# danielreardon/scintools

Hardware: NVIDIA B200
Metric: theta-theta eta-trials/sec on 4096x8192 dynspec (higher is better)
Workload: dtype f32

## Files before the change

### scintools_b200/csrc/api.cu

```cuda
#include <stdarg.h>
#include <string.h>

#include <vector>

#include "../../include/scint_b200.h"
#include "common.cuh"
#include "thth.cuh"

namespace sb {

static thread_local char g_err[512] = "";
static void* g_ws[8] = {nullptr};
static size_t g_ws_bytes[8] = {0};
static int g_sms = 148;

void set_error(const char* fmt, ...) {
    va_list ap;
    va_start(ap, fmt);
    vsnprintf(g_err, sizeof(g_err), fmt, ap);
    va_end(ap);
}
const char* last_error() { return g_err; }
int num_sms() { return g_sms; }

static long long g_launches = 0;
void count_launch() { ++g_launches; }

struct ProfPair { int id; cudaEvent_t a, b; };
static bool g_prof_on = false;
static std::vector<ProfPair> g_prof_pending;
static std::vector<cudaEvent_t> g_prof_pool;
static cudaEvent_t g_prof_open[PROF_COUNT];

static cudaEvent_t prof_event() {
    if (!g_prof_pool.empty()) {
        cudaEvent_t e = g_prof_pool.back();
        g_prof_pool.pop_back();
        return e;
    }
    cudaEvent_t e;
    cudaEventCreate(&e);
    return e;
}
void prof_begin(int id, cudaStream_t st) {
    if (!g_prof_on) return;
    g_prof_open[id] = prof_event();
    cudaEventRecord(g_prof_open[id], st);
}
void prof_end(int id, cudaStream_t st) {
    if (!g_prof_on) return;
    cudaEvent_t b = prof_event();
    cudaEventRecord(b, st);
    g_prof_pending.push_back({id, g_prof_open[id], b});
}

void* workspace(int slot, size_t bytes) {
    if (slot < 0 || slot >= 8) return nullptr;
    if (bytes <= g_ws_bytes[slot] && g_ws[slot]) return g_ws[slot];
    if (g_ws[slot]) {
        cudaDeviceSynchronize();
        cudaFree(g_ws[slot]);
        g_ws[slot] = nullptr;
        g_ws_bytes[slot] = 0;
    }
    size_t want = (bytes + (size_t(1) << 20) - 1) & ~((size_t(1) << 20) - 1);
    void* p = nullptr;
    cudaError_t e = cudaMalloc(&p, want);
    if (e != cudaSuccess) {
        set_error("workspace slot %d: cudaMalloc(%zu) -> %s", slot, want,
                  cudaGetErrorString(e));
        cudaGetLastError();
        return nullptr;
    }
    g_ws[slot] = p;
    g_ws_bytes[slot] = want;
    return p;
}

void workspace_release() {
    cudaDeviceSynchronize();
    for (int i = 0; i < 8; ++i) {
        if (g_ws[i]) cudaFree(g_ws[i]);
        g_ws[i] = nullptr;
        g_ws_bytes[i] = 0;
    }
}

int eta_sweep(const ThthGeom& g, const double* th_host, const double* d_etas,
              int neta, double tol, int max_iter, double* d_eigs,
              int* d_status, int* d_nred, int* d_iters, cudaStream_t st);
int thth_map(const ThthGeom& g, double eta, int hermitian, float2* d_out,
             int* d_tau_inv, int* d_fd_inv, unsigned char* d_pnts,
             unsigned char* d_th_pnts, int* d_err, cudaStream_t st);

int sspec(const float* dyn, int nf, int nt, const float* wt, const float* wf,
          double swt, double swf, int prewhite, int halve, int db,
          const float* pd1, const float* pd2, float* sec, cudaStream_t st,
          int noshift = 0);
int conj_spectrum(const float* dyn, int nf, int nt, int npad, float pad_value,
                  const unsigned char* rowmask, int half, long pitch, int ncols_keep,
                  float2* CS, cudaStream_t st);
int acf(const float* dyn, int nf, int nt, int subtract_mean, int normalise,
        float* out, cudaStream_t st);
int acf_sspec(const float* dyn, int nf, int nt, const float* wt, const float* wf,
              double swt, double swf, int normalise, float* out, cudaStream_t st);
void twiddle_release();
struct SimParams {
    int nx, ny;
    double dx, dy, alpha, ar, psi, inner, consp;
};
int sim_weights(const SimParams& p, double* w, cudaStream_t st);
int sim_screen(int nx, int ny, const double* w, const double* n1, const double* n2,
               unsigned long long seed, double* xyp, cudaStream_t st);
int sim_intensity(int nx, int ny, int nf, const double* xyp, const double* scales_host,
                  double ffconx, double ffcony, float2* spe_t, float* xyi,
                  cudaStream_t st);

template <typename A, typename B>
__global__ void convert_kernel(const A* __restrict__ a, B* __restrict__ b, long long n) {
    for (long long i = (long long)blockIdx.x * blockDim.x + threadIdx.x; i < n;
         i += (long long)gridDim.x * blockDim.x)
        b[i] = (B)a[i];
}

struct ThinGeom {
    ThthGeom g;
    const double* th2;
    int n2;
    double tau_max;
    double center_cut;
    int power;
};
int thin_sweep(const ThinGeom& t, const double* d_eta1, const double* d_eta2, int neta,
               double tol, int max_iter, double* d_sv, int* d_status, int* d_n1, int* d_n2,
               int* d_iters, cudaStream_t st);
int thin_map(const ThinGeom& t, double e1, double e2, float2* d_out, int* d_err,
             cudaStream_t st);

int rev_map(const float2* thth, int n, const double* th_dev, double eta, double tau0,
            double dtau, int ntau, double fd0, double dfd, int nfd, int hermitian,
            float2* recov, cudaStream_t st);
int herm_eigvec(const float2* A, int n, int ld, double tol, int max_iter, double* w_dev,
                float2* V_dev, int* info_dev, cudaStream_t st);
int ifft2_c2c(const float2* in, int n0, int n1, int centred, int crop0, int crop1,
              double scale, int real_only, void* out, cudaStream_t st);

int gerchberg_saxton(float2* W, const float* amp, const unsigned char* rowmask, int n0, int n1,
                     int niter, cudaStream_t st);

int conj_spectrum_bound(const float* dyn, int nf, int nt, int npad, float pad_value, float* out,
                        cudaStream_t st);
int norm_sspec_rows(const float* sspec, int nr, int nc, const double* fdop, const double* tdel,
                    double eta, double maxnormfac, const double* fdopnew, int nq, float* out,
                    double* power, cudaStream_t st);
int norm_sspec_avg(const float* norm, int nr, int nq, const double* weights, double* avg,
                   cudaStream_t st);
int scale_dyn_lambda(const float* dyn, int nf, int nt, int flip, const float* a,
                     const float* cp, const float* inv, const float* g, float p0, float pn,
                     const int* idx, const float4* W, int nlam, float* out, cudaStream_t st);

static int to_geom(const sb_thth_geom* in, ThthGeom* g) {
    SB_ARG(in != nullptr);
    SB_ARG(in->ntau > 0 && in->nfd > 0);
    SB_ARG(in->th_cents != nullptr && in->th_cents_host != nullptr);
    SB_ARG(in->n_th > 0);
    g->cs = (const float2*)in->cs;
    g->ntau = in->ntau;
    g->nfd = in->nfd;
    g->tau0 = in->tau0;
    g->dtau = in->dtau;
    g->half_dtau = in->dtau / 2;
    g->tau_absmax = in->tau_absmax;
    g->fd0 = in->fd0;
    g->dfd = in->dfd;
    g->half_dfd = in->dfd / 2;
    g->inv_dtau = 1.0 / in->dtau;
    g->inv_dfd = 1.0 / in->dfd;
    g->fd_half = in->fd_half;
    g->th = in->th_cents;
    g->n = in->n_th;
    g->coherent = in->coherent;
    g->cs_half = in->cs_half;
    g->cs_valid_cols = in->cs_half ? in->cs_valid_cols : 0;
    g->cs_bound = in->cs_bound;
    g->cs_pitch = in->cs_half ? in->cs_pitch : (in->cs_pitch > 0 ? in->cs_pitch : in->nfd);
    SB_ARG(!in->cs_half || (in->cs_pitch >= in->nfd / 2 + 1 && in->nfd % 2 == 0));
    return SB_OK;
}

}

extern "C" {

int sb_abi_version(void) { return 2; }
const char* sb_last_error(void) { return sb::last_error(); }

int sb_init(int device) {
    SB_CUDA(cudaSetDevice(device));
    SB_CUDA(cudaFree(0));
    cudaDeviceProp prop;
    SB_CUDA(cudaGetDeviceProperties(&prop, device));
    if (prop.major != 10) {
        sb::set_error("device %d is sm_%d%d; libscint_b200 is sm_100a only",
                      device, prop.major, prop.minor);
        return SB_ERR_UNSUPPORTED;
    }
    sb::g_sms = prop.multiProcessorCount;
    return SB_OK;
}

int64_t sb_launch_count(void) { return sb::g_launches; }

int sb_profile_enable(int32_t on) {
    sb::g_prof_on = on != 0;
    return SB_OK;
}

int sb_profile_collect(double* ms_host, int32_t* count_host, int32_t n) {
    SB_ARG(ms_host && count_host && n >= sb::PROF_COUNT);
    for (int i = 0; i < n; ++i) { ms_host[i] = 0.0; count_host[i] = 0; }
    SB_CUDA(cudaDeviceSynchronize());
    for (auto& p : sb::g_prof_pending) {
        float ms = 0.f;
        cudaEventElapsedTime(&ms, p.a, p.b);
        ms_host[p.id] += ms;
        count_host[p.id] += 1;
        sb::g_prof_pool.push_back(p.a);
        sb::g_prof_pool.push_back(p.b);
    }
    sb::g_prof_pending.clear();
    return SB_OK;
}

int sb_release(void) {
// ... 199 lines not shown
```

### scintools_b200/csrc/common.cuh

```cuda
#pragma once
#ifndef SB_HOST_EMU
#include <cuda_runtime.h>
#include <stdint.h>
#include <stdio.h>

#include "../../include/scint_b200.h"

namespace sb {

void set_error(const char* fmt, ...);
const char* last_error();

void* workspace(int slot, size_t bytes);
void workspace_release();
int num_sms();

enum ProfId { PROF_CS_ROWS = 0, PROF_CS_COLA, PROF_CS_COLB, PROF_THTH_PREP,
              PROF_THTH_BUILD, PROF_THTH_EIG, PROF_SSPEC, PROF_ACF, PROF_SIM_SCREEN,
              PROF_SIM_FREQ, PROF_COUNT };
void prof_begin(int id, cudaStream_t st);
void prof_end(int id, cudaStream_t st);
struct ProfScope {
    int id; cudaStream_t st;
    ProfScope(int i, cudaStream_t s) : id(i), st(s) { prof_begin(id, st); }
    ~ProfScope() { prof_end(id, st); }
};

#define SB_CUDA(call)                                                        \
    do {                                                                     \
        cudaError_t _e = (call);                                             \
        if (_e != cudaSuccess) {                                             \
            sb::set_error("%s:%d %s -> %s", __FILE__, __LINE__, #call,       \
                          cudaGetErrorString(_e));                           \
            return SB_ERR_CUDA;                                              \
        }                                                                    \
    } while (0)

void count_launch();

#define SB_LAUNCH_CHECK()                                                    \
    do {                                                                     \
        sb::count_launch();                                                  \
        cudaError_t _e = cudaGetLastError();                                 \
        if (_e != cudaSuccess) {                                             \
            sb::set_error("%s:%d launch -> %s", __FILE__, __LINE__,          \
                          cudaGetErrorString(_e));                           \
            return SB_ERR_CUDA;                                              \
        }                                                                    \
    } while (0)

#define SB_ARG(cond)                                                         \
    do {                                                                     \
        if (!(cond)) {                                                       \
            sb::set_error("%s:%d bad argument: %s", __FILE__, __LINE__,      \
                          #cond);                                            \
            return SB_ERR_ARG;                                               \
        }                                                                    \
    } while (0)

}
#endif

#ifdef SB_HOST_EMU
#define SB_SHARED static
#else
#define SB_SHARED __shared__
#endif

namespace sb {

__device__ __forceinline__ float warp_sum(float v) {
#pragma unroll
    for (int o = 16; o > 0; o >>= 1) v += __shfl_xor_sync(0xffffffffu, v, o);
    return v;
}
__device__ __forceinline__ double warp_sum(double v) {
#pragma unroll
    for (int o = 16; o > 0; o >>= 1) v += __shfl_xor_sync(0xffffffffu, v, o);
    return v;
}

__device__ __forceinline__ double floor_div_exact(double a, double b) {
    if (b > 0.0 && isfinite(a)) {
        double q = floor(__ddiv_rn(a, b));
        double r = __fma_rn(-q, b, a);
        if (r < 0.0) q -= 1.0;
        else if (r >= b) q += 1.0;
        return q;
    }
    if (b == 0.0) return __ddiv_rn(a, b);
    double mod = fmod(a, b);
    double div = __ddiv_rn(__dsub_rn(a, mod), b);
    if (mod != 0.0) {
        if ((b < 0.0) != (mod < 0.0)) div -= 1.0;
    }
    if (div != 0.0) {
        double fl = floor(div);
        if (div - fl > 0.5) fl += 1.0;
        return fl;
    }
    return copysign(0.0, __ddiv_rn(a, b));
}

__device__ __forceinline__ double floor_div_fast(double a, double b, double inv_b) {
    double q = floor(a * inv_b);
    if (b > 0.0 && fabs(q) < 1.0e15) {
        double r = __fma_rn(-q, b, a);
        if (r < 0.0) q -= 1.0;
        else if (r >= b) q += 1.0;
        return q;
    }
    return floor_div_exact(a, b);
}

}
```

### scintools_b200/csrc/thth.cu

```cuda
#include <float.h>
#include <limits.h>
#include <math.h>
#include <stdlib.h>

#include <type_traits>

#include "bf16_pack.cuh"
#include "lanczos.cuh"
#include "thth.cuh"
#include "tma.cuh"

namespace sb {

#ifndef SB_HOST_EMU
int eig_cluster_launch(const float2* d_M, int ld, int n_max, const int* d_nred, int e0,
                       int nb, double* d_eigs, int* d_status, int* d_iters, double tol,
                       double etol, int max_iter, cudaStream_t st);

int eig_half_launch(const float2* d_M, const unsigned* d_Mb, int ld, const int* d_nred, int e0,
                    int nb, double* d_eigs, int* d_status, int* d_iters, double tol, double etol,
                    int max_iter, bool tensor, cudaStream_t st);

#endif

enum { ST_OK = 0, ST_INDEX_ERROR = 1, ST_ZERO_START = 2, ST_TOO_SMALL = 4,
       ST_NOT_CONVERGED = 8 };

__global__ void thth_prep_kernel(ThthGeom g, const double* __restrict__ etas,
                                 int neta, int ld, int* __restrict__ idx,
                                 int* __restrict__ nred) {
    int e = blockIdx.x;
    if (e >= neta) return;
    double eta = etas[e];
    int lane = threadIdx.x;
    int base = 0;
    int* out = idx + (size_t)e * ld;
    for (int k0 = 0; k0 < g.n; k0 += 32) {
        int k = k0 + lane;
        bool keep = false;
        if (k < g.n) {
            double t = g.th[k];
            keep = (__dmul_rn(__dmul_rn(t, t), eta) < g.tau_absmax) &&
                   (fabs(t) < g.fd_half);
        }
        unsigned m = __ballot_sync(0xffffffffu, keep);
        if (keep) out[base + __popc(m & ((1u << lane) - 1u))] = k;
        base += __popc(m);
    }
    if (lane == 0) nred[e] = base;
}

__global__ void thth_indexerr_kernel(ThthGeom g, const double* __restrict__ etas,
                                     int* __restrict__ status) {
    int e = blockIdx.y;
    double eta = etas[e];
    long long total = (long long)g.n * g.n;
    bool bad = false;
    for (long long p = (long long)blockIdx.x * blockDim.x + threadIdx.x;
         p < total; p += (long long)gridDim.x * blockDim.x) {
        int i = (int)(p / g.n), j = (int)(p % g.n);
        ThthPoint pt = thth_point(g, eta, g.th[j], g.th[i]);
        bad |= pt.index_error;
    }
    if (__any_sync(0xffffffffu, bad) && (threadIdx.x & 31) == 0)
        atomicOr(status + e, ST_INDEX_ERROR);
}

#define SB_BUILD_EB 8

__device__ __forceinline__ unsigned pack_f16x2(float2 v) {
#ifdef SB_HOST_EMU
    const __half2 h = __floats2half2_rn(v.x, v.y);
    return (unsigned)h.x | ((unsigned)h.y << 16);
#else
    unsigned r;
    asm("cvt.rn.f16x2.f32 %0, %1, %2;" : "=r"(r) : "f"(v.y), "f"(v.x));
    return r;
#endif
}

__global__ void cs_absmax_kernel(const float2* __restrict__ cs, long long rows, long long ncols,
                                 long long pitch, unsigned* __restrict__ out) {
    float m = 0.f;
    const long long per_row4 = ncols >> 1;
    const long long total = rows * per_row4;
    for (long long i = (long long)blockIdx.x * blockDim.x + threadIdx.x; i < total;
         i += (long long)gridDim.x * blockDim.x) {
        const long long r = i / per_row4, c = i - r * per_row4;
        const float4 q = __ldg(reinterpret_cast<const float4*>(cs + r * pitch) + c);
        m = fmaxf(fmaxf(fmaxf(fabsf(q.x), fabsf(q.y)), fmaxf(fabsf(q.z), fabsf(q.w))), m);
    }
    if (ncols & 1) {
        for (long long r = (long long)blockIdx.x * blockDim.x + threadIdx.x; r < rows;
             r += (long long)gridDim.x * blockDim.x) {
            const float2 q = __ldg(cs + r * pitch + ncols - 1);
            m = fmaxf(fmaxf(fabsf(q.x), fabsf(q.y)), m);
        }
    }
    if (!(m == m)) m = 3.0e38f;
    m = fminf(m, 3.0e38f);
#pragma unroll
    for (int o = 16; o > 0; o >>= 1) m = fmaxf(m, __shfl_xor_sync(0xffffffffu, m, o));
    if ((threadIdx.x & 31) == 0) atomicMax(out, __float_as_uint(m));
}

template <int PACK, int ROWS, typename OFF>
__global__ void __launch_bounds__(32 * (32 / ROWS), ROWS == 8 ? 5 : 4)
thth_build_kernel(ThthGeom g, const double* __restrict__ etas, int eta0, int nbatch,
                  int ld, const int* __restrict__ idx,
                  const int* __restrict__ nred, float2* __restrict__ M,
                  unsigned* __restrict__ Mb, const unsigned* __restrict__ absmax, float span) {
    constexpr int TY = 32 / ROWS;
    int p = blockIdx.y, ta = 0;
    const int T = ld / 32;
    while (p >= T - ta) { p -= T - ta; ++ta; }
    const int tb = ta + p;
    const int tx = threadIdx.x, ty = threadIdx.y;
    const int b = tb * 32 + tx;
    const double ntau_d = (double)g.ntau;
    const long long hfd = g.nfd / 2;
    int cj = -2;
    double thj = 0.0;
    int ci[ROWS];
    double dk[ROWS];
    int col[ROWS];
    unsigned conj = 0u;
    float wk[ROWS];
#pragma unroll
    for (int k = 0; k < ROWS; ++k) { ci[k] = -2; dk[k] = 0.0; col[k] = -1; wk[k] = 0.f; }
    const int e_end = min(nbatch, (int)(blockIdx.x + 1) * SB_BUILD_EB);
    __shared__ float s_hscale[SB_BUILD_EB];
    if (PACK != 0) {
        const int lin = ty * 32 + tx;
        if (lin < SB_BUILD_EB) {
            const int e = blockIdx.x * SB_BUILD_EB + lin;
            float hs = 1.f;
            if (e < e_end) {
                const float seta = sqrtf((float)(2.0 * etas[eta0 + e]));
                const float bound = __uint_as_float(*absmax) * seta * sqrtf(span);
                if (bound > 0.f && bound < 3.0e38f) {
                    const float q = 32768.f / bound;
                    hs = q >= 1.1754944e-38f ? __uint_as_float(__float_as_uint(q) & 0x7f800000u) : 1.1754944e-38f;
                }
            }
            s_hscale[lin] = hs;
        }
        __syncthreads();
    }
    const unsigned foff0 = (unsigned)(ta * 32 + ty) * (unsigned)ld + (unsigned)b;
    const unsigned frow = (unsigned)TY * (unsigned)ld;
    const unsigned woff0 = ((unsigned)(2 * ta) * (unsigned)(ld >> 3) + (unsigned)(b >> 3)) * 128u +
                           (unsigned)ty * 8u;
    for (int e = blockIdx.x * SB_BUILD_EB; e < e_end; ++e) {
        const int n = nred[eta0 + e];
        if (tb * 32 >= n) continue;
        const double eta = etas[eta0 + e];
        const int* id = idx + (size_t)(eta0 + e) * ld;
        const int j = b < n ? id[b] : -1;
        if (j != cj) {
            cj = j;
            thj = j >= 0 ? g.th[j] : 0.0;
#pragma unroll
            for (int k = 0; k < ROWS; ++k) ci[k] = -2;
        }
        const float seta = sqrtf((float)(2.0 * eta));
        float2* Me = M + (size_t)e * ld * ld;
        const float hscale = PACK != 0 ? s_hscale[e - blockIdx.x * SB_BUILD_EB] : 1.f;
        OFF off[ROWS];
        unsigned hit = 0u;
#pragma unroll
        for (int k = 0; k < ROWS; ++k) {
            const int la = ty + TY * k;
            off[k] = 0;
            if (ta == tb && tx < la) continue;
            const int a = ta * 32 + la;
            const int i = a < n ? id[a] : -1;
            if (i != ci[k]) {
                ci[k] = i;
                col[k] = -1;
                conj &= ~(1u << k);
                wk[k] = 0.f;
                dk[k] = 0.0;
                if (i >= 0 && j > i && i + j != g.n - 1) {
                    const double th1 = thj, th2 = g.th[i];
                    dk[k] = __dsub_rn(__dmul_rn(th1, th1), __dmul_rn(th2, th2));
                    const double bb = __dadd_rn(__dsub_rn(__dsub_rn(th1, th2), g.fd0), g.half_dfd);
                    const double fqd = floor_div_fast(bb, g.dfd, g.inv_dfd);
                    const long long fq = (fqd == fqd && fabs(fqd) < 9.0e18) ? (long long)fqd : LLONG_MIN;
                    wk[k] = sqrtf((float)fabs(th2 - th1));
                    if (fq < g.nfd && !(fq < -g.nfd)) {
                        const long long fi = fq < 0 ? fq + g.nfd : fq;
                        if (!g.cs_half) col[k] = (int)fi;
                        else if (fi >= hfd) col[k] = (int)(fi - hfd);
                        else if (fi == 0) col[k] = (int)hfd;
                        else { col[k] = (int)(hfd - fi); conj |= 1u << k; }
                    }
                }
            }
            if (col[k] >= 0) {
                const double aa = __dadd_rn(__dsub_rn(__dmul_rn(eta, dk[k]), g.tau0), g.half_dtau);
                const double tqd = floor_div_fast(aa, g.dtau, g.inv_dtau);
                if (tqd > 0.0 && tqd < ntau_d) {
                    const int tq = (int)tqd;
                    const int r = (conj >> k) & 1u ? (int)g.ntau - tq : tq;
                    off[k] = (OFF)r * (OFF)g.cs_pitch + (OFF)col[k];
                    hit |= 1u << k;
                }
            }
        }
        float2 val[ROWS];
#pragma unroll
        for (int k = 0; k < ROWS; ++k) val[k] = __ldg(g.cs + off[k]);
#pragma unroll
        for (int k = 0; k < ROWS; ++k) {
            const int la = ty + TY * k;
            const bool low = ta == tb && tx < la;
            float2 v = make_float2(0.f, 0.f);
            if (!low) {
                if (col[k] >= 0) {
                    if ((hit >> k) & 1u) {
                        v = val[k];
                        if ((conj >> k) & 1u) v.y = -v.y;
                        if (!g.coherent) v = make_float2(hypotf(v.x, v.y), 0.f);
                    }
                    const float wf = seta * wk[k];
                    v.x *= wf;
                    v.y *= wf;
                    if (!(fabsf(v.x) <= 3.402823466e+38f) || !(fabsf(v.y) <= 3.402823466e+38f)) {
                        v.x = nan_to_num(v.x);
                        v.y = nan_to_num(v.y);
                    }
                }
                const unsigned o = foff0 + (unsigned)k * frow;
                Me[o] = v;
                if (PACK == 1) Mb[(size_t)e * ld * ld + o] = pack_f16x2(make_float2(v.x * hscale, v.y * hscale));
            }
            if (PACK == 2) {
                const unsigned h = low ? 0u : pack_f16x2(make_float2(v.x * hscale, v.y * hscale));
                const int i8 = tx & 7, s0 = (tx & ~7) + 2 * (i8 & 3);
                const unsigned ha = __shfl_sync(0xffffffffu, h, s0);
                const unsigned hb = __shfl_sync(0xffffffffu, h, s0 + 1);
                const unsigned word = i8 < 4 ? ((ha & 0xffffu) | (hb << 16)) : ((ha >> 16) | (hb & 0xffff0000u));
                if (!(ta == tb && (tx >> 4) < (la >> 4))) {
                    unsigned* Mw = Mb + (size_t)e * ld * ld;
                    const unsigned swz = (unsigned)(((la & 15) >> 2) & 1) << 2;
                    Mw[woff0 + (unsigned)(la >> 4) * (unsigned)(ld >> 3) * 128u + (unsigned)((la & 15) - ty) * 8u +
                       ((unsigned)i8 ^ swz)] = word;
                }
            }
        }
    }
}

template <int THREADS, bool TMA, int NST, bool FAST = false>
__global__ void __launch_bounds__(THREADS)
thth_eig_kernel(const float2* __restrict__ Mbase, int ld,
                const int* __restrict__ nred, int eta0,
                double* __restrict__ eigs, int* __restrict__ status,
                int* __restrict__ iters, double tol, double etol, int max_iter, int nb) {
    extern __shared__ __align__(128) unsigned char smem_raw[];
    constexpr int NW = THREADS / 32;
    LanczosShared& S = *reinterpret_cast<LanczosShared*>(smem_raw);
    float2* v = reinterpret_cast<float2*>(smem_raw + sizeof(LanczosShared));
    float2* vp = v + ld;
    float2* w = vp + ld;
    float2* u = w + ld;
    float4* stages = reinterpret_cast<float4*>(u + ld);
    float2* part = reinterpret_cast<float2*>(stages);
    unsigned long long* mbar = reinterpret_cast<unsigned long long*>(
        reinterpret_cast<unsigned char*>(stages) +
        (TMA ? (size_t)NW * NST * 4096 : (size_t)NW * 4096));
    const int tid = threadIdx.x, lane = tid & 31, warp = tid >> 5;
    if (TMA) {
        if (tid == 0) {
            for (int i = 0; i < NW * NST; ++i) mbar_init(mbar + i, 1);
            fence_mbarrier_init();
        }
    }
    unsigned gi = 0, gc = 0;
    for (int e = blockIdx.x; e < nb; e += gridDim.x) {
    __syncthreads();
    const int n = nred[eta0 + e];
    const float2* M = Mbase + (size_t)e * ld * ld;
    const double qnan = __longlong_as_double(0x7ff8000000000000LL);

    if (status[eta0 + e] & ST_INDEX_ERROR) {
        if (tid == 0) { eigs[eta0 + e] = qnan; iters[eta0 + e] = 0; }
        continue;
    }
    if (n < 3) {
        if (tid == 0) {
            eigs[eta0 + e] = qnan; iters[eta0 + e] = 0;
            status[eta0 + e] |= ST_TOO_SMALL;
        }
        continue;
    }
    const int h = n / 2;
    double part0 = 0.0;
    for (int c = tid; c < ld; c += THREADS) {
        float2 x = make_float2(0.f, 0.f);
        if (c < n && c > h) x = M[(size_t)h * ld + c];
        else if (c < h) { x = M[(size_t)c * ld + h]; x.y = -x.y; }
        v[c] = x;
        vp[c] = make_float2(0.f, 0.f);
        part0 += (double)x.x * x.x + (double)x.y * x.y;
    }
    part0 = warp_sum(part0);
    if (lane == 0) S.red[0][warp] = part0;
    if (tid == 0) {
        S.done = 0; S.lo = 0.0; S.theta = 0.0; S.res = 0.0; S.m_lo2 = 0; S.lo2 = 0.0;
        S.next_check = 1; S.m_last = 0; S.beta2[0] = 0.0;
    }
    __syncthreads();
    double nrm2 = 0.0;
    for (int k = 0; k < NW; ++k) nrm2 += S.red[0][k];
    if (!(nrm2 > 0.0) || !isfinite(nrm2)) {
        if (tid == 0) {
            eigs[eta0 + e] = qnan; iters[eta0 + e] = 0;
            status[eta0 + e] |= ST_ZERO_START;
        }
        continue;
    }
    {
        float s = (float)(1.0 / sqrt(nrm2));
        for (int c = tid; c < ld; c += THREADS) { v[c].x *= s; v[c].y *= s; }
    }
    __syncthreads();

    const int ncol4 = (n + 1) >> 1;
    const int nchunk = (n + 511) / 512;
    float4* mystage = stages + (size_t)warp * NST * 256;
    unsigned long long* mybar = mbar + warp * NST;
    float beta_prev = 0.f;
    int m = 0;
    for (int it = 0; it < max_iter; ++it) {
        for (int c = tid; c < ld; c += THREADS) w[c] = make_float2(0.f, 0.f);
        __syncthreads();
        if constexpr (TMA) {
            float4 yc[8];
#pragma unroll
            for (int j = 0; j < 8; ++j) yc[j] = make_float4(0.f, 0.f, 0.f, 0.f);
            const int K = (n - 2 >= warp) ? (n - 2 - warp) / NW + 1 : 0;
            const bool tail = ncol4 < 256;
            const float4* v4 = reinterpret_cast<const float4*>(v);
            for (int k = 0; k < NST && k < K; ++k) {
                const int st = gi % NST;
                ++gi;
                if (lane == 0) {
                    const int a = warp + NW * k;
                    const int c_lo = (a + 1) & ~1;
                    const unsigned bytes = (unsigned)(2 * ncol4 - c_lo) * 8u;
                    mbar_expect_tx(mybar + st, bytes);
                    bulk_g2s(reinterpret_cast<float2*>(mystage + st * 256) + c_lo,
                             M + (size_t)a * ld + c_lo, bytes, mybar + st);
                }
            }
            int k = 0;
            auto run_rows = [&](auto JSc) {
                constexpr int JS = decltype(JSc)::value;
                for (; k < K && ((warp + NW * k + 1) >> 6) == JS; ++k) {
                    const int a = warp + NW * k;
                    const int first4 = (a + 1) >> 1;
                    const float2 xa = v[a];
                    const int st = gc % NST;
                    const unsigned par = (gc / NST) & 1u;
                    ++gc;
                    while (!mbar_try_wait(mybar + st, par)) {}
                    const float4* sg = mystage + st * 256;
                    float rxa = 0.f, rxb = 0.f, rya = 0.f, ryb = 0.f;
#pragma unroll
                    for (int j = JS; j < 8; ++j) {
                        const int c4 = lane + 32 * j;
                        float4 q = sg[c4];
                        bool ok = (j > JS) || (c4 >= first4);
                        if (tail) ok = ok && (c4 < ncol4);
                        if (!ok) q = make_float4(0.f, 0.f, 0.f, 0.f);
                        float4 x = make_float4(0.f, 0.f, 0.f, 0.f);
                        if (ok) x = v4[c4];
                        rxa = fmaf(q.x, x.x, rxa); rxb = fmaf(-q.y, x.y, rxb);
                        rxa = fmaf(q.z, x.z, rxa); rxb = fmaf(-q.w, x.w, rxb);
                        rya = fmaf(q.x, x.y, rya); ryb = fmaf(q.y, x.x, ryb);
                        rya = fmaf(q.z, x.w, rya); ryb = fmaf(q.w, x.z, ryb);
                        yc[j].x = fmaf(q.x, xa.x, yc[j].x); yc[j].x = fmaf(q.y, xa.y, yc[j].x);
                        yc[j].y = fmaf(q.x, xa.y, yc[j].y); yc[j].y = fmaf(-q.y, xa.x, yc[j].y);
                        yc[j].z = fmaf(q.z, xa.x, yc[j].z); yc[j].z = fmaf(q.w, xa.y, yc[j].z);
                        yc[j].w = fmaf(q.z, xa.y, yc[j].w); yc[j].w = fmaf(-q.w, xa.x, yc[j].w);
                    }
                    __syncwarp();
                    const bool more = k + NST < K;
                    const int st2 = gi % NST;
                    if (more) ++gi;
                    if (lane == 0 && more) {
                        const int a2 = warp + NW * (k + NST);
                        const int c_lo = (a2 + 1) & ~1;
                        const unsigned bytes = (unsigned)(2 * ncol4 - c_lo) * 8u;
                        mbar_expect_tx(mybar + st2, bytes);
                        bulk_g2s(reinterpret_cast<float2*>(mystage + st2 * 256) + c_lo,
                                 M + (size_t)a2 * ld + c_lo, bytes, mybar + st2);
                    }
                    const float rx = rxa + rxb, ry = rya + ryb;
// ... 162 lines not shown
        if (warp == 0 && (m >= S.next_check || last || !(beta > 0.0))) {
            if (FAST) lanczos_check_fast(S, m, tol, etol);
            else lanczos_check(S, m, tol, etol);
        }
        __syncthreads();
        if (S.done || !isfinite(alpha)) break;
        const float ib = (float)(1.0 / beta);
        for (int c = tid; c < n; c += THREADS) {
            float2 x = w[c];
            vp[c] = v[c];
            v[c] = make_float2(x.x * ib, x.y * ib);
        }
        beta_prev = (float)beta;
        __syncthreads();
    }
    if (tid == 0) {
        eigs[eta0 + e] = fabs(S.theta);
        iters[eta0 + e] = m;
        if (!S.done) status[eta0 + e] |= ST_NOT_CONVERGED;
    }
    }
}

__global__ void thth_map_kernel(ThthGeom g, double eta, int hermitian,
                                float2* __restrict__ out,
                                int* __restrict__ tau_inv,
                                int* __restrict__ fd_inv,
                                unsigned char* __restrict__ pnts,
                                int* __restrict__ err) {
    long long total = (long long)g.n * g.n;
    for (long long p = (long long)blockIdx.x * blockDim.x + threadIdx.x;
         p < total; p += (long long)gridDim.x * blockDim.x) {
        int i = (int)(p / g.n), j = (int)(p % g.n);
        double thi = g.th[i], thj = g.th[j];
        ThthPoint pt = thth_point(g, eta, thj, thi);
        if (pt.index_error) atomicOr(err, ST_INDEX_ERROR);
        if (tau_inv) tau_inv[p] = (int)max(min(pt.tq, (long long)INT_MAX), (long long)INT_MIN);
        if (fd_inv) fd_inv[p] = (int)max(min(pt.fq, (long long)INT_MAX), (long long)INT_MIN);
        if (pnts) pnts[p] = pt.pnt ? 1 : 0;
        if (!out) continue;
        float2 v;
        if (!hermitian) {
            v = thth_value(g, eta, thj, thi, pt);
        } else if (i == j || i + j == g.n - 1) {
            v = make_float2(0.f, 0.f);
        } else if (j > i) {
            v = thth_value(g, eta, thj, thi, pt);
            v.x = nan_to_num(v.x);
            v.y = nan_to_num(v.y);
        } else {
            ThthPoint pu = thth_point(g, eta, thi, thj);
            v = thth_value(g, eta, thi, thj, pu);
            v.x = nan_to_num(v.x);
            v.y = -nan_to_num(v.y);
        }
        out[p] = v;
    }
}

#ifndef SB_HOST_EMU
static bool lower_check_needed(const ThthGeom& g, const double* th_host) {
    double tmin = th_host[0], tmax = th_host[0];
    for (int k = 1; k < g.n; ++k) {
        tmin = th_host[k] < tmin ? th_host[k] : tmin;
        tmax = th_host[k] > tmax ? th_host[k] : tmax;
    }
    double worst = floor(((tmin - tmax) - g.fd0 + g.half_dfd) / g.dfd) - 2.0;
    return !(worst >= -(double)g.nfd);
}

int eta_sweep(const ThthGeom& g, const double* th_host, const double* d_etas,
              int neta, double tol, int max_iter, double* d_eigs,
              int* d_status, int* d_nred, int* d_iters, cudaStream_t st) {
    if (neta <= 0) return SB_OK;
    if (max_iter <= 0 || max_iter > SB_LANCZOS_MAXIT) max_iter = SB_LANCZOS_MAXIT;
    const int ld = (g.n + 31) / 32 * 32;
    if (ld > 4096) {
        set_error("theta-theta grid of %d centres exceeds the supported 4096", g.n);
        return SB_ERR_UNSUPPORTED;
    }
    int* d_idx = (int*)workspace(1, (size_t)neta * ld * sizeof(int));
    if (!d_idx) return SB_ERR_NOMEM;
    SB_CUDA(cudaMemsetAsync(d_status, 0, neta * sizeof(int), st));
    prof_begin(PROF_THTH_PREP, st);
    thth_prep_kernel<<<neta, 32, 0, st>>>(g, d_etas, neta, ld, d_idx, d_nred);
    prof_end(PROF_THTH_PREP, st);
    SB_LAUNCH_CHECK();
    if (lower_check_needed(g, th_host)) {
        dim3 grid(64, neta);
        thth_indexerr_kernel<<<grid, 256, 0, st>>>(g, d_etas, d_status);
        SB_LAUNCH_CHECK();
    }
    const size_t per = (size_t)ld * ld * sizeof(float2);
    unsigned long long slab = 3ull << 30;
    if (const char* ev = getenv("SB_SWEEP_SLAB_MB")) {
        const long mb = atol(ev);
        if (mb > 0) slab = (unsigned long long)mb << 20;
    }
    int batch = (int)(slab / per);
    if (batch < 1) batch = 1;
    if (batch > neta) batch = neta;
    float2* d_M = (float2*)workspace(2, per * batch);
    if (!d_M) return SB_ERR_NOMEM;
    const bool mixed = (ld <= 512) && !getenv("SB_EIG_FP32") && !getenv("SB_EIG_CLUSTER") &&
                       !getenv("SB_EIG_PERSIST") && !getenv("SB_EIG_NO_TMA");
    unsigned* d_Mb = nullptr;
    if (mixed) {
        d_Mb = (unsigned*)workspace(6, per / 2 * batch);
        if (!d_Mb) return SB_ERR_NOMEM;
    }
    const int T = ld / 32;
    const int npairs = T * (T + 1) / 2;
    constexpr int TT = 256, TS = 2;
    constexpr int DT = 512;
    const bool use_tma = (ld <= 512) && !getenv("SB_EIG_NO_TMA");
    const size_t smem = sizeof(LanczosShared) + 4 * (size_t)ld * sizeof(float2) +
                        (use_tma ? (size_t)(TT / 32) * TS * 4096 + 512
                                 : (size_t)(DT / 32) * 4096 + 512);
    int persist = 0;
    if (const char* ev = getenv("SB_EIG_PERSIST")) persist = atoi(ev);
    constexpr int PS = 4;
    const size_t smem_p = sizeof(LanczosShared) + 4 * (size_t)ld * sizeof(float2) +
                          (size_t)(TT / 32) * PS * 4096 + 512;
    if (use_tma && persist > 0)
        SB_CUDA(cudaFuncSetAttribute(thth_eig_kernel<TT, true, PS, true>,
                                     cudaFuncAttributeMaxDynamicSharedMemorySize, (int)smem_p));
    if (use_tma)
        SB_CUDA(cudaFuncSetAttribute(thth_eig_kernel<TT, true, TS>,
                                     cudaFuncAttributeMaxDynamicSharedMemorySize, (int)smem));
    else
        SB_CUDA(cudaFuncSetAttribute(thth_eig_kernel<DT, false, 1>,
                                     cudaFuncAttributeMaxDynamicSharedMemorySize, (int)smem));
    unsigned* d_absmax = nullptr;
    float span = 0.f;
    if (mixed) {
        d_absmax = (unsigned*)workspace(0, 64 * sizeof(double)) + 32;
        if (!d_absmax) return SB_ERR_NOMEM;
        if (g.cs_bound) {
            SB_CUDA(cudaMemcpyAsync(d_absmax, g.cs_bound, sizeof(float), cudaMemcpyDeviceToDevice, st));
        } else {
            SB_CUDA(cudaMemsetAsync(d_absmax, 0, sizeof(unsigned), st));
            const long long ncols = g.cs_half ? (g.cs_valid_cols > 0 ? g.cs_valid_cols : g.nfd / 2 + 1)
                                              : g.nfd;
            cs_absmax_kernel<<<num_sms() * 8, 256, 0, st>>>(g.cs, g.ntau, ncols, g.cs_pitch, d_absmax);
            SB_LAUNCH_CHECK();
        }
        double tmin = th_host[0], tmax = th_host[0];
        for (int k = 1; k < g.n; ++k) {
            tmin = th_host[k] < tmin ? th_host[k] : tmin;
            tmax = th_host[k] > tmax ? th_host[k] : tmax;
        }
        span = (float)((tmax - tmin) * 1.0001);
    }
    for (int e0 = 0; e0 < neta; e0 += batch) {
        int nb = neta - e0 < batch ? neta - e0 : batch;
        static const int BR = (getenv("SB_BUILD_ROWS") && atoi(getenv("SB_BUILD_ROWS")) == 8) ? 8 : 4;
        const bool tensor = mixed && BR == 4 && !getenv("SB_EIG_NO_TC");
        dim3 grid((nb + SB_BUILD_EB - 1) / SB_BUILD_EB, npairs), block(32, 32 / BR);
        prof_begin(PROF_THTH_BUILD, st);
        const bool small = (unsigned long long)g.ntau * (unsigned long long)g.cs_pitch < (1ull << 32);
#define SB_BUILD_LAUNCH(PACK, ROWS, OFF, MB, AM, SP)                                        \
        thth_build_kernel<PACK, ROWS, OFF><<<grid, block, 0, st>>>(g, d_etas, e0, nb, ld, d_idx, \
                                                                   d_nred, d_M, MB, AM, SP)
        if (BR == 8) {
            if (mixed && small) SB_BUILD_LAUNCH(1, 8, unsigned, d_Mb, d_absmax, span);
            else if (mixed) SB_BUILD_LAUNCH(1, 8, size_t, d_Mb, d_absmax, span);
            else if (small) SB_BUILD_LAUNCH(0, 8, unsigned, nullptr, nullptr, 0.f);
            else SB_BUILD_LAUNCH(0, 8, size_t, nullptr, nullptr, 0.f);
        } else if (tensor) {
            if (small) SB_BUILD_LAUNCH(2, 4, unsigned, d_Mb, d_absmax, span);
            else SB_BUILD_LAUNCH(2, 4, size_t, d_Mb, d_absmax, span);
        } else {
            if (mixed && small) SB_BUILD_LAUNCH(1, 4, unsigned, d_Mb, d_absmax, span);
            else if (mixed) SB_BUILD_LAUNCH(1, 4, size_t, d_Mb, d_absmax, span);
            else if (small) SB_BUILD_LAUNCH(0, 4, unsigned, nullptr, nullptr, 0.f);
            else SB_BUILD_LAUNCH(0, 4, size_t, nullptr, nullptr, 0.f);
        }
#undef SB_BUILD_LAUNCH
        prof_end(PROF_THTH_BUILD, st);
        SB_LAUNCH_CHECK();
        prof_begin(PROF_THTH_EIG, st);
        int rc = mixed ? eig_half_launch(d_M, d_Mb, ld, d_nred, e0, nb, d_eigs, d_status,
                                         d_iters, tol, 2e-7, max_iter, tensor, st)
                       : 0;
        if (rc == 0)
            rc = eig_cluster_launch(d_M, ld, g.n, d_nred, e0, nb, d_eigs, d_status, d_iters,
                                    tol, 2e-7, max_iter, st);
        if (rc < 0) return rc;
        if (rc > 0) {
        } else if (use_tma && persist > 0)
            thth_eig_kernel<TT, true, PS, true><<<persist < nb ? persist : nb, TT, smem_p, st>>>(
                d_M, ld, d_nred, e0, d_eigs, d_status, d_iters, tol, 2e-7, max_iter, nb);
        else if (use_tma)
            thth_eig_kernel<TT, true, TS><<<nb, TT, smem, st>>>(
                d_M, ld, d_nred, e0, d_eigs, d_status, d_iters, tol, 2e-7, max_iter, nb);
        else
            thth_eig_kernel<DT, false, 1><<<nb, DT, smem, st>>>(
                d_M, ld, d_nred, e0, d_eigs, d_status, d_iters, tol, 2e-7, max_iter, nb);
        prof_end(PROF_THTH_EIG, st);
        SB_LAUNCH_CHECK();
    }
    return SB_OK;
}

__global__ void thth_mask_kernel(ThthGeom g, double eta,
                                 unsigned char* __restrict__ mask) {
    int k = blockIdx.x * blockDim.x + threadIdx.x;
    if (k >= g.n) return;
    double t = g.th[k];
    mask[k] = ((__dmul_rn(__dmul_rn(t, t), eta) < g.tau_absmax) &&
               (fabs(t) < g.fd_half)) ? 1 : 0;
}

int thth_map(const ThthGeom& g, double eta, int hermitian, float2* d_out,
             int* d_tau_inv, int* d_fd_inv, unsigned char* d_pnts,
             unsigned char* d_th_pnts, int* d_err, cudaStream_t st) {
    if (d_th_pnts) {
        thth_mask_kernel<<<(g.n + 255) / 256, 256, 0, st>>>(g, eta, d_th_pnts);
        SB_LAUNCH_CHECK();
    }
    if (!d_err) return SB_OK;
    SB_CUDA(cudaMemsetAsync(d_err, 0, sizeof(int), st));
    long long total = (long long)g.n * g.n;
    int blocks = (int)((total + 255) / 256);
    if (blocks > 148 * 16) blocks = 148 * 16;
    thth_map_kernel<<<blocks, 256, 0, st>>>(g, eta, hermitian, d_out, d_tau_inv,
                                            d_fd_inv, d_pnts, d_err);
    SB_LAUNCH_CHECK();
    return SB_OK;
}

#endif

}
```

Baseline: 208,500.

## Compact referenced conjugate-spectrum columns into L2-resident buffer for theta-theta build

Before the eta sweep, the code marks which conjugate-spectrum columns any theta pair can touch, prefix-scans them into a slot map, and gathers those columns into a column-major compact buffer sized to fit in three quarters of L2. The build kernel then reads from this buffer through remapped offsets, with an evict_last L2 policy on loads and evict_first on matrix stores. The goal is to turn scattered strided gathers from the large spectrum into L2-resident accesses. It adds three setup kernels, extra workspace, and a fallback to the original path when the compacted columns exceed capacity.

```diff
diff --git a/scintools_b200/csrc/api.cu b/scintools_b200/csrc/api.cu
--- a/scintools_b200/csrc/api.cu
+++ b/scintools_b200/csrc/api.cu
@@ -10,8 +10,8 @@
 namespace sb {
 
 static thread_local char g_err[512] = "";
-static void* g_ws[8] = {nullptr};
-static size_t g_ws_bytes[8] = {0};
+static void* g_ws[SB_WORKSPACE_SLOTS] = {nullptr};
+static size_t g_ws_bytes[SB_WORKSPACE_SLOTS] = {0};
 static int g_sms = 148;
 
 void set_error(const char* fmt, ...) {
@@ -55,7 +55,7 @@
 }
 
 void* workspace(int slot, size_t bytes) {
-    if (slot < 0 || slot >= 8) return nullptr;
+    if (slot < 0 || slot >= SB_WORKSPACE_SLOTS) return nullptr;
     if (bytes <= g_ws_bytes[slot] && g_ws[slot]) return g_ws[slot];
     if (g_ws[slot]) {
         cudaDeviceSynchronize();
@@ -79,7 +79,7 @@
 
 void workspace_release() {
     cudaDeviceSynchronize();
-    for (int i = 0; i < 8; ++i) {
+    for (int i = 0; i < SB_WORKSPACE_SLOTS; ++i) {
         if (g_ws[i]) cudaFree(g_ws[i]);
         g_ws[i] = nullptr;
         g_ws_bytes[i] = 0;
diff --git a/scintools_b200/csrc/common.cuh b/scintools_b200/csrc/common.cuh
--- a/scintools_b200/csrc/common.cuh
+++ b/scintools_b200/csrc/common.cuh
@@ -11,6 +11,7 @@
 void set_error(const char* fmt, ...);
 const char* last_error();
 
+constexpr int SB_WORKSPACE_SLOTS = 10;
 void* workspace(int slot, size_t bytes);
 void workspace_release();
 int num_sms();
diff --git a/scintools_b200/csrc/thth.cu b/scintools_b200/csrc/thth.cu
--- a/scintools_b200/csrc/thth.cu
+++ b/scintools_b200/csrc/thth.cu
@@ -79,6 +79,158 @@
 #endif
 }
 
+__device__ __forceinline__ unsigned long long l2_policy_evict_first() {
+#ifdef SB_HOST_EMU
+    return 0ull;
+#else
+    unsigned long long p;
+    asm("createpolicy.fractional.L2::evict_first.b64 %0, 1.0;" : "=l"(p));
+    return p;
+#endif
+}
+__device__ __forceinline__ unsigned long long l2_policy_evict_last() {
+#ifdef SB_HOST_EMU
+    return 0ull;
+#else
+    unsigned long long p;
+    asm("createpolicy.fractional.L2::evict_last.b64 %0, 1.0;" : "=l"(p));
+    return p;
+#endif
+}
+__device__ __forceinline__ unsigned long long l2_policy_evict_normal() {
+#ifdef SB_HOST_EMU
+    return 0ull;
+#else
+    unsigned long long p;
+    asm("createpolicy.fractional.L2::evict_normal.b64 %0, 1.0;" : "=l"(p));
+    return p;
+#endif
+}
+__device__ __forceinline__ float2 ldg_l2(const float2* p, unsigned long long pol) {
+#ifdef SB_HOST_EMU
+    (void)pol;
+    return *p;
+#else
+    float2 v;
+    asm("ld.global.nc.L2::cache_hint.v2.f32 {%0, %1}, [%2], %3;"
+        : "=f"(v.x), "=f"(v.y) : "l"(p), "l"(pol));
+    return v;
+#endif
+}
+__device__ __forceinline__ void st_l2(float2* p, float2 v, unsigned long long pol) {
+#ifdef SB_HOST_EMU
+    (void)pol;
+    *p = v;
+#else
+    asm volatile("st.global.L2::cache_hint.v2.f32 [%0], {%1, %2}, %3;"
+                 :: "l"(p), "f"(v.x), "f"(v.y), "l"(pol));
+#endif
+}
+__device__ __forceinline__ void st_l2(unsigned* p, unsigned v, unsigned long long pol) {
+#ifdef SB_HOST_EMU
+    (void)pol;
+    *p = v;
+#else
+    asm volatile("st.global.L2::cache_hint.b32 [%0], %1, %2;" :: "l"(p), "r"(v), "l"(pol));
+#endif
+}
+
+__device__ __forceinline__ int thth_pair_column(const ThthGeom& g, double th1, double th2,
+                                                bool* conj) {
+    *conj = false;
+    const double bb = __dadd_rn(__dsub_rn(__dsub_rn(th1, th2), g.fd0), g.half_dfd);
+    const double fqd = floor_div_fast(bb, g.dfd, g.inv_dfd);
+    const long long fq = (fqd == fqd && fabs(fqd) < 9.0e18) ? (long long)fqd : LLONG_MIN;
+    if (!(fq < g.nfd) || fq < -g.nfd) return -1;
+    const long long hfd = g.nfd / 2;
+    const long long fi = fq < 0 ? fq + g.nfd : fq;
+    if (!g.cs_half) return (int)fi;
+    if (fi >= hfd) return (int)(fi - hfd);
+    if (fi == 0) return (int)hfd;
+    *conj = true;
+    return (int)(hfd - fi);
+}
+
+__global__ void thth_colmark_kernel(ThthGeom g, int* __restrict__ slot_of_col) {
+    const long long total = (long long)g.n * g.n;
+    for (long long p = (long long)blockIdx.x * blockDim.x + threadIdx.x; p < total;
+         p += (long long)gridDim.x * blockDim.x) {
+        const int i = (int)(p / g.n), j = (int)(p % g.n);
+        if (j <= i || i + j == g.n - 1) continue;
+        bool cj;
+        const int c = thth_pair_column(g, g.th[j], g.th[i], &cj);
+        if (c >= 0) slot_of_col[c] = 1;
+    }
+}
+
+__global__ void thth_colscan_kernel(int ncols, int cap, int* __restrict__ cmap) {
+    int* slot_of_col = cmap + 2;
+    int* col_of_slot = cmap + 2 + ncols;
+    const int t = threadIdx.x, nt = blockDim.x, lane = t & 31, w = t >> 5;
+    const int per = (ncols + nt - 1) / nt;
+    const int c0 = min(ncols, t * per), c1 = min(ncols, c0 + per);
+    int cnt = 0;
+    for (int c = c0; c < c1; ++c) cnt += slot_of_col[c] != 0;
+    int x = cnt;
+#pragma unroll
+    for (int o = 1; o < 32; o <<= 1) {
+        const int y = __shfl_sync(0xffffffffu, x, lane >= o ? lane - o : lane);
+        if (lane >= o) x += y;
+    }
+    SB_SHARED int s_w[32];
+    if (lane == 31) s_w[w] = x;
+    __syncthreads();
+    if (w == 0) {
+        int v = lane < (nt >> 5) ? s_w[lane] : 0;
+#pragma unroll
+        for (int o = 1; o < 32; o <<= 1) {
+            const int y = __shfl_sync(0xffffffffu, v, lane >= o ? lane - o : lane);
+            if (lane >= o) v += y;
+        }
+        s_w[lane] = v;
+    }
+    __syncthreads();
+    int s = x - cnt + (w > 0 ? s_w[w - 1] : 0);
+    for (int c = c0; c < c1; ++c) {
+        if (slot_of_col[c]) {
+            slot_of_col[c] = s;
+            col_of_slot[s++] = c;
+        } else {
+            slot_of_col[c] = -1;
+        }
+    }
+    if (t == nt - 1) {
+        cmap[1] = s;
+        cmap[0] = s <= cap ? 1 : 0;
+    }
+}
+
+#define SB_COMPACT_ROWS 64
+__global__ void __launch_bounds__(256)
+thth_cs_compact_kernel(ThthGeom g, const int* __restrict__ cmap,
+                       const int* __restrict__ col_of_slot, float2* __restrict__ C) {
+    SB_SHARED float2 tile[32][SB_COMPACT_ROWS + 1];
+    if (!cmap[0]) return;
+    const int nslots = cmap[1];
+    const int s0 = blockIdx.y * 32;
+    if (s0 >= nslots) return;
+    const long long r0 = (long long)blockIdx.x * SB_COMPACT_ROWS;
+    const int lane = threadIdx.x & 31, warp = threadIdx.x >> 5;
+    const int ns = min(32, nslots - s0);
+    const unsigned long long pol = l2_policy_evict_first();
+    const int c = lane < ns ? col_of_slot[s0 + lane] : 0;
+    for (int k = warp; k < SB_COMPACT_ROWS; k += 8) {
+        const long long r = r0 + k;
+        if (lane < ns && r < g.ntau) tile[lane][k] = ldg_l2(g.cs + r * g.cs_pitch + c, pol);
+    }
+    __syncthreads();
+    for (int s = warp; s < ns; s += 8)
+        for (int k = lane; k < SB_COMPACT_ROWS; k += 32) {
+            const long long r = r0 + k;
+            if (r < g.ntau) C[(long long)(s0 + s) * g.ntau + r] = tile[s][k];
+        }
+}
+
 __global__ void cs_absmax_kernel(const float2* __restrict__ cs, long long rows, long long ncols,
                                  long long pitch, unsigned* __restrict__ out) {
     float m = 0.f;
@@ -104,12 +256,13 @@
     if ((threadIdx.x & 31) == 0) atomicMax(out, __float_as_uint(m));
 }
 
-template <int PACK, int ROWS, typename OFF>
+template <int PACK, int ROWS, typename OFF, bool COMPACT = false>
 __global__ void __launch_bounds__(32 * (32 / ROWS), ROWS == 8 ? 5 : 4)
 thth_build_kernel(ThthGeom g, const double* __restrict__ etas, int eta0, int nbatch,
                   int ld, const int* __restrict__ idx,
                   const int* __restrict__ nred, float2* __restrict__ M,
-                  unsigned* __restrict__ Mb, const unsigned* __restrict__ absmax, float span) {
+                  unsigned* __restrict__ Mb, const unsigned* __restrict__ absmax, float span,
+                  const float2* __restrict__ cc = nullptr, const int* __restrict__ cmap = nullptr) {
     constexpr int TY = 32 / ROWS;
     int p = blockIdx.y, ta = 0;
     const int T = ld / 32;
@@ -118,7 +271,13 @@
     const int tx = threadIdx.x, ty = threadIdx.y;
     const int b = tb * 32 + tx;
     const double ntau_d = (double)g.ntau;
-    const long long hfd = g.nfd / 2;
+    const bool cmp = COMPACT && cmap[0];
+    const float2* src = cmp ? cc : g.cs;
+    unsigned long long pol_ld = 0ull, pol_st = 0ull;
+    if (COMPACT) {
+        pol_ld = cmp ? l2_policy_evict_last() : l2_policy_evict_normal();
+        pol_st = l2_policy_evict_first();
+    }
     int cj = -2;
     double thj = 0.0;
     int ci[ROWS];
@@ -129,7 +288,7 @@
 #pragma unroll
     for (int k = 0; k < ROWS; ++k) { ci[k] = -2; dk[k] = 0.0; col[k] = -1; wk[k] = 0.f; }
     const int e_end = min(nbatch, (int)(blockIdx.x + 1) * SB_BUILD_EB);
-    __shared__ float s_hscale[SB_BUILD_EB];
+    SB_SHARED float s_hscale[SB_BUILD_EB];
     if (PACK != 0) {
         const int lin = ty * 32 + tx;
         if (lin < SB_BUILD_EB) {
@@ -184,17 +343,12 @@
                 if (i >= 0 && j > i && i + j != g.n - 1) {
                     const double th1 = thj, th2 = g.th[i];
                     dk[k] = __dsub_rn(__dmul_rn(th1, th1), __dmul_rn(th2, th2));
-                    const double bb = __dadd_rn(__dsub_rn(__dsub_rn(th1, th2), g.fd0), g.half_dfd);
-                    const double fqd = floor_div_fast(bb, g.dfd, g.inv_dfd);
-                    const long long fq = (fqd == fqd && fabs(fqd) < 9.0e18) ? (long long)fqd : LLONG_MIN;
                     wk[k] = sqrtf((float)fabs(th2 - th1));
-                    if (fq < g.nfd && !(fq < -g.nfd)) {
-                        const long long fi = fq < 0 ? fq + g.nfd : fq;
-                        if (!g.cs_half) col[k] = (int)fi;
-                        else if (fi >= hfd) col[k] = (int)(fi - hfd);
-                        else if (fi == 0) col[k] = (int)hfd;
-                        else { col[k] = (int)(hfd - fi); conj |= 1u << k; }
-                    }
+                    bool cg;
+                    int c = thth_pair_column(g, th1, th2, &cg);
+                    if (cmp && c >= 0) c = cmap[2 + c];
+                    col[k] = c;
+                    if (cg) conj |= 1u << k;
                 }
             }
             if (col[k] >= 0) {
@@ -203,14 +357,15 @@
                 if (tqd > 0.0 && tqd < ntau_d) {
                     const int tq = (int)tqd;
                     const int r = (conj >> k) & 1u ? (int)g.ntau - tq : tq;
-                    off[k] = (OFF)r * (OFF)g.cs_pitch + (OFF)col[k];
+                    if (cmp) off[k] = (OFF)col[k] * (OFF)g.ntau + (OFF)r;
+                    else off[k] = (OFF)r * (OFF)g.cs_pitch + (OFF)col[k];
                     hit |= 1u << k;
                 }
             }
         }
         float2 val[ROWS];
 #pragma unroll
-        for (int k = 0; k < ROWS; ++k) val[k] = __ldg(g.cs + off[k]);
+        for (int k = 0; k < ROWS; ++k) val[k] = COMPACT ? ldg_l2(src + off[k], pol_ld) : __ldg(g.cs + off[k]);
 #pragma unroll
         for (int k = 0; k < ROWS; ++k) {
             const int la = ty + TY * k;
@@ -232,8 +387,13 @@
                     }
                 }
                 const unsigned o = foff0 + (unsigned)k * frow;
-                Me[o] = v;
-                if (PACK == 1) Mb[(size_t)e * ld * ld + o] = pack_f16x2(make_float2(v.x * hscale, v.y * hscale));
+                if (COMPACT) st_l2(Me + o, v, pol_st);
+                else Me[o] = v;
+                if (PACK == 1) {
+                    const unsigned h = pack_f16x2(make_float2(v.x * hscale, v.y * hscale));
+                    if (COMPACT) st_l2(Mb + (size_t)e * ld * ld + o, h, pol_st);
+                    else Mb[(size_t)e * ld * ld + o] = h;
+                }
             }
             if (PACK == 2) {
                 const unsigned h = low ? 0u : pack_f16x2(make_float2(v.x * hscale, v.y * hscale));
@@ -244,8 +404,10 @@
                 if (!(ta == tb && (tx >> 4) < (la >> 4))) {
                     unsigned* Mw = Mb + (size_t)e * ld * ld;
                     const unsigned swz = (unsigned)(((la & 15) >> 2) & 1) << 2;
-                    Mw[woff0 + (unsigned)(la >> 4) * (unsigned)(ld >> 3) * 128u + (unsigned)((la & 15) - ty) * 8u +
-                       ((unsigned)i8 ^ swz)] = word;
+                    unsigned* pw = Mw + woff0 + (unsigned)(la >> 4) * (unsigned)(ld >> 3) * 128u +
+                                   (unsigned)((la & 15) - ty) * 8u + ((unsigned)i8 ^ swz);
+                    if (COMPACT) st_l2(pw, word, pol_st);
+                    else *pw = word;
                 }
             }
         }
@@ -714,16 +876,50 @@
         }
         span = (float)((tmax - tmin) * 1.0001);
     }
+    const long long ncols = g.cs_half ? g.nfd / 2 + 1 : g.nfd;
+    int dev = 0, l2 = 0;
+    SB_CUDA(cudaGetDevice(&dev));
+    SB_CUDA(cudaDeviceGetAttribute(&l2, cudaDevAttrL2CacheSize, dev));
+    long long cap = (long long)l2 / 4 * 3 / (g.ntau * (long long)sizeof(float2));
+    if (cap > ncols) cap = ncols;
+    if (cap > 65535LL * 32) cap = 65535LL * 32;
+    int* d_cmap = nullptr;
+    float2* d_C = nullptr;
+    if (cap >= 1 && ncols < (INT_MAX - 2) / 2) {
+        d_C = (float2*)workspace(8, (size_t)cap * g.ntau * sizeof(float2));
+        if (!d_C) return SB_ERR_NOMEM;
+        d_cmap = (int*)workspace(9, (size_t)(2 + 2 * ncols) * sizeof(int));
+        if (!d_cmap) return SB_ERR_NOMEM;
+    }
     for (int e0 = 0; e0 < neta; e0 += batch) {
         int nb = neta - e0 < batch ? neta - e0 : batch;
         static const int BR = (getenv("SB_BUILD_ROWS") && atoi(getenv("SB_BUILD_ROWS")) == 8) ? 8 : 4;
         const bool tensor = mixed && BR == 4 && !getenv("SB_EIG_NO_TC");
         dim3 grid((nb + SB_BUILD_EB - 1) / SB_BUILD_EB, npairs), block(32, 32 / BR);
         prof_begin(PROF_THTH_BUILD, st);
+        if (d_cmap && e0 == 0) {
+            SB_CUDA(cudaMemsetAsync(d_cmap, 0, (size_t)(2 + ncols) * sizeof(int), st));
+            const long long pairs = (long long)g.n * g.n;
+            thth_colmark_kernel<<<(int)((pairs + 255) / 256 < 1024 ? (pairs + 255) / 256 : 1024), 256, 0, st>>>(
+                g, d_cmap + 2);
+            SB_LAUNCH_CHECK();
+            thth_colscan_kernel<<<1, 1024, 0, st>>>((int)ncols, (int)cap, d_cmap);
+            SB_LAUNCH_CHECK();
+            const dim3 cgrid((unsigned)((g.ntau + SB_COMPACT_ROWS - 1) / SB_COMPACT_ROWS),
+                             (unsigned)((cap + 31) / 32));
+            thth_cs_compact_kernel<<<cgrid, 256, 0, st>>>(g, d_cmap, d_cmap + 2 + ncols, d_C);
+            SB_LAUNCH_CHECK();
+        }
         const bool small = (unsigned long long)g.ntau * (unsigned long long)g.cs_pitch < (1ull << 32);
-#define SB_BUILD_LAUNCH(PACK, ROWS, OFF, MB, AM, SP)                                        \
-        thth_build_kernel<PACK, ROWS, OFF><<<grid, block, 0, st>>>(g, d_etas, e0, nb, ld, d_idx, \
-                                                                   d_nred, d_M, MB, AM, SP)
+#define SB_BUILD_LAUNCH(PACK, ROWS, OFF, MB, AM, SP)                                             \
+        do {                                                                                      \
+            if (d_cmap)                                                                           \
+                thth_build_kernel<PACK, ROWS, OFF, true><<<grid, block, 0, st>>>(                 \
+                    g, d_etas, e0, nb, ld, d_idx, d_nred, d_M, MB, AM, SP, d_C, d_cmap);          \
+            else                                                                                  \
+                thth_build_kernel<PACK, ROWS, OFF><<<grid, block, 0, st>>>(                       \
+                    g, d_etas, e0, nb, ld, d_idx, d_nred, d_M, MB, AM, SP);                       \
+        } while (0)
         if (BR == 8) {
             if (mixed && small) SB_BUILD_LAUNCH(1, 8, unsigned, d_Mb, d_absmax, span);
             else if (mixed) SB_BUILD_LAUNCH(1, 8, size_t, d_Mb, d_absmax, span);
```

Result: no change. 209,300 (median of 6 runs) (+0.4%).
